# LCSL/nys-koop-lqr

Hardware: AMD Instinct MI355X
Metric: Nyström-Koopman fits/sec (K_nm build + A,B,C solve), N=1e5 m=2000 d=384 (higher is better)
Workload: dtype f64

## Files before the change

nys_koop_lqr_amd/csrc/nk_api.hip:

```cpp
#include "nk_common.h"
#include "nk_plant.h"

#include <cmath>
#include <cstdarg>
#include <cstdio>
#include <cstring>
#include <chrono>
#include <cstdlib>
#include <algorithm>
#include <condition_variable>
#include <functional>
#include <mutex>
#include <set>
#include <thread>

namespace nk {

static thread_local std::string g_err;

void set_error(const char* fmt, ...) {
  char buf[1024];
  va_list ap;
  va_start(ap, fmt);
  vsnprintf(buf, sizeof(buf), fmt, ap);
// ... 1357 lines not shown
      double *Res = nullptr, *ResT = nullptr, *partial = nullptr;
      const int64_t ldt_ = nr + (nr & 1);
      NK_TRY(arena_alloc_t(ctx, (size_t)nr * mq, &Res));
      NK_TRY(arena_alloc_t(ctx, (size_t)mq * ldt_, &ResT));
      NK_TRY(arena_alloc_t(ctx, (size_t)2 * refine_partial_blocks(), &partial));
      CholSys y = sys[q];
      y.R = ResT; y.ldr = ldt_; y.nrhs = nr;
      for (int step = 0; step < refine_steps; ++step) {
        NK_TRY(launch_resid_dd(ctx, Xq, mq, Pq, mq, Rq, mq, Res, mq, nr, mq));
        NK_TRY(launch_transpose(ctx, Res, mq, ResT, ldt_, nr, mq));
        NK_TRY(cholesky_solve_pair(ctx, &y, 1));
        NK_TRY(launch_transpose(ctx, ResT, ldt_, Res, mq, mq, nr));
        NK_TRY(launch_refine_apply(ctx, Res, mq, Xq, mq, nr, mq, step, refine_state + 4 * q, partial));
      }
      NK_HIP(hipMemcpyAsync(ctx->h_scalars + 16 + 4 * q, refine_state + 4 * q, 4 * sizeof(double), hipMemcpyDeviceToHost,
                            ctx->stream));
      arena_release(ctx, mk);
      refined[q] = -1;
      redo_products = true;
    }
  }
  {
    const int vr = sqrtm_verdict(ctx, &splan, &it, &resid);
    if (vr == NK_SQRT_RETRY && splan.flow_gave_up) {
      ChainOnly chain(ctx);
      SqrtPlan again;
      again.lambda_min_hint = splan.lambda_min_hint;
      NK_TRY(sqrtm_prepare(ctx, Kj, m, m, &again));
      NK_TRY(sqrtm_finish(ctx, &again, mdl->S, mdl->Sinv));
      NK_HIP(hipStreamSynchronize(ctx->stream));
      const int vr2 = sqrtm_verdict(ctx, &again, &it, &resid);
      if (vr2 == NK_SQRT_RETRY) {
        count_event(CNT_SQRT_RETRY);
        NK_TRY(sqrtm_spd_coupled(ctx, Kj, m, m, mdl->S, mdl->Sinv, &it, &resid));
      } else {
        NK_TRY(vr2);
      }
      NK_TRY(sqrt_products());
      redo_products = true;
    } else if (vr == NK_SQRT_RETRY) {
      count_event(CNT_SQRT_RETRY);
      NK_TRY(sqrtm_spd_coupled(ctx, Kj, m, m, mdl->S, mdl->Sinv, &it, &resid));
      NK_TRY(sqrt_products());
      redo_products = true;
    } else {
      NK_TRY(vr);
    }
// ... 1207 lines not shown
```

nys_koop_lqr_amd/csrc/nk_common.h:

```cpp
#pragma once
#include <hip/hip_runtime.h>
#include <stdint.h>
#include <stddef.h>
#include <string>
#include <vector>

#include "nyskoop.h"
#include "nk_lockstep.h"

namespace nk {

void set_error(const char* fmt, ...);

#define NK_HIP(call)                                                                         \
  do {                                                                                       \
    hipError_t e_ = (call);                                                                  \
    if (e_ != hipSuccess) {                                                                  \
      nk::set_error("%s failed: %s (%s:%d)", #call, hipGetErrorString(e_), __FILE__, __LINE__); \
      return e_ == hipErrorOutOfMemory ? NK_ERR_OOM : NK_ERR_HIP;                            \
    }                                                                                        \
  } while (0)

#define NK_TRY(call)            \
  do {                          \
// ... 166 lines not shown
  const double z = s * s;
  const double w = z * z;
  const double t1 = w * (Lg2 + w * (Lg4 + w * Lg6));
  const double t2 = z * (Lg1 + w * (Lg3 + w * (Lg5 + w * Lg7)));
  const double R = t2 + t1;
  if (((hx - 0x6147a) | (0x6b851 - hx)) > 0) {
    const double hfsq = 0.5 * f * f;
    return k == 0 ? f - (hfsq - s * (hfsq + R)) : dk * ln2_hi - ((hfsq - (s * (hfsq + R) + dk * ln2_lo)) - f);
  }
  return k == 0 ? f - s * (f - R) : dk * ln2_hi - ((s * (f - R) - dk * ln2_lo) - f);
}
__host__ __device__ __forceinline__ double tps_value(double r2) {
#pragma clang fp contract(off)
  return r2 > 0.0 ? r2 * log_pos(sqrt(r2)) : 0.0;
}

nk_group* group_new(int device, int size);
void group_attach(nk_group* g, int slot, nk_ctx* c);
void group_detach(nk_ctx* c);
int group_enter(nk_ctx* c);
int group_leave(nk_ctx* c);
void group_stats(nk_ctx* c, uint64_t out[4]);
enum { CNT_CHAIN_GIVEUP = 0, CNT_JACOBI_GIVEUP = 1, CNT_RANK_TRUNCATED = 2, CNT_SQRT_RETRY = 3, CNT_REFINED = 4,
       CNT_CHOL_FLOW_GIVEUP = 5, CNT_CHOL_FLOW = 6, CNT_N = 7 };
void count_event(int which);
uint64_t read_counter(int which);
hipError_t real_stream_sync(hipStream_t s);
hipError_t real_event_sync(hipEvent_t e);

int arena_reset(nk_ctx* ctx);
ArenaMark arena_mark(nk_ctx* ctx);
void arena_release(nk_ctx* ctx, ArenaMark mk);
int arena_alloc(nk_ctx* ctx, size_t bytes, void** out);
template <typename T>
inline int arena_alloc_t(nk_ctx* ctx, size_t count, T** out) {
  return arena_alloc(ctx, count * sizeof(T), reinterpret_cast<void**>(out));
}
bool is_device_ptr(const void* p);

int launch_kmat(nk_ctx* ctx, int ktype, const double* A, int64_t lda, int64_t nA, const double* B, int64_t ldb,
                int64_t nB, int d, const double* winv, double sigma0, double* out, int64_t ldo);

enum { TRI_FULL = 0, TRI_UPPER_MIRROR = 1, TRI_LOWER = 2 };
struct GemmOpts {
  int tri = TRI_FULL;
  int splitk = 0;
};
// ... 24 lines not shown
                               const TnSkip* skip = nullptr);
int launch_max_abs_rowsum(nk_ctx* ctx, const double* M, int64_t ldm, int n, double* d_out);
int launch_colsum_sqdiff(nk_ctx* ctx, const double* P, int64_t ldp, const double* Y, int64_t ldy, int64_t rows,
                         int cols, double* d_colsum);

int sqrtm_spd(nk_ctx* ctx, const double* P, int64_t ldp, int m, double* S, double* Sinv, int* iters, double* resid);
struct SqrtPlan {
  const double* P = nullptr;
  int64_t ldp = 0;
  int m = 0;
  double* W = nullptr;
  double* Linv = nullptr;
  double* X0 = nullptr;
  double* X0t = nullptr;
  double* d_sc = nullptr;
  ArenaMark mark{0, 0};
  bool deferred = false;
  int rc = 0, iters = 0, kmax = 0;
  double resid = 0.0;
  double lambda_min_hint = 0.0;
  bool early = false;
  int info_slot = 2;
  bool flow_gave_up = false;
  hipEvent_t pause_event = nullptr;
  int pause_step = -1;
};
constexpr int NK_SQRT_RETRY = 1;
int sqrtm_spd_coupled(nk_ctx* ctx, const double* P, int64_t ldp, int m, double* S, double* Sinv, int* iters, double* resid);
int sqrtm_prepare(nk_ctx* ctx, const double* P, int64_t ldp, int m, SqrtPlan* plan);
int sqrtm_finish(nk_ctx* ctx, SqrtPlan* plan, double* S, double* Sinv);
int sqrtm_verdict(nk_ctx* ctx, SqrtPlan* plan, int* iters, double* resid);
int cholesky_lower(nk_ctx* ctx, double* P, int64_t ldp, int m, double* Linv );
int cholesky_solve(nk_ctx* ctx, const double* L, int64_t ldl, int m, const double* Linv, double* R, int64_t ldr,
                   int nrhs);
struct CholSys {
  double* P = nullptr;
  int64_t ldp = 0;
  int m = 0;
  int extra = 0;
  bool backward = true;
  double* Linv = nullptr;
  double* pivlog = nullptr;
  double* R = nullptr;
  int64_t ldr = 0;
  int nrhs = 0;
};
int cholesky_lower_pair(nk_ctx* ctx, const CholSys* sys, int nsys);
int cholesky_lower_pair_async(nk_ctx* ctx, const CholSys* sys, int nsys);
int cholesky_check_pair(nk_ctx* ctx, const CholSys* sys, int nsys);
int cholesky_solve_pair(nk_ctx* ctx, const CholSys* sys, int nsys);
int cholesky_aug_pair_async(nk_ctx* ctx, const CholSys* sys, int nsys, hipEvent_t pause = nullptr, int pause_step = -1);
constexpr int CHOL_NB = 64;
constexpr int CHOL_WS = 2 * CHOL_NB * CHOL_NB + 8;
constexpr double CHOL_FIX_KAPPA = 8.0 * CHOL_NB;
// ... 63 lines not shown
  const double* A = nullptr;
  const double* B = nullptr;
  double* C = nullptr;
  int64_t lda = 0, ldb = 0, ldc = 0;
  int M = 0, N = 0;
  int tri = TRI_FULL;
  int ktrim = 0;
  double alpha = 1.0, beta = 0.0;
  double* Ct = nullptr;
  int64_t ldct = 0;
  const double* A_even = nullptr;
  const double* B_even = nullptr;
  double* Caff = nullptr;
  double aff_a = 0.0, aff_c = 0.0;
};
struct TnSkip {
  const double* state = nullptr;
  int step = 0;
  const double* select = nullptr;
  double* resid_partials = nullptr;
  int* resid_count = nullptr;
};
bool tn_fast_ok(const TnProblem& p);
struct TnProblemF {
  const float* A = nullptr;
  const float* B = nullptr;
  double* C = nullptr;
  int64_t lda = 0, ldb = 0, ldc = 0;
  int M = 0, N = 0;
  int tri = TRI_FULL;
  double beta = 0.0;
};
bool tnf_fast_ok(const TnProblemF& p);
int launch_gemm_tn_f32_multi(nk_ctx* ctx, const TnProblemF* probs, int nprob, int64_t K, int splitk ,
                             float* ms_kernel = nullptr, bool sync_timing = true);
int prep_rows_f32(nk_ctx* ctx, const double* X, int64_t ldx, int64_t rows, int d, const double* winv, const double* center,
                  float* Xt, int64_t ldt, float* sq);
int launch_cvt_f64_f32(nk_ctx* ctx, const double* src, int64_t lds_, float* dst, int64_t ldd, int64_t rows, int cols);
int launch_kmat_gram_f32(nk_ctx* ctx, int ktype, const float* At, int64_t ldat, const float* sqa, int64_t nA, const float* Bt,
                         int64_t ldbt, const float* sqb, int64_t nB, int d, double sigma0, float* out, int64_t ldo);
int launch_gemm_tn_multi(nk_ctx* ctx, const TnProblem* probs, int nprob, int64_t K, int splitk ,
                         float* ms_kernel = nullptr, bool sync_timing = true, const TnSkip* skip = nullptr);
int launch_transpose(nk_ctx* ctx, const double* src, int64_t lds, double* dst, int64_t ldd, int rows, int cols);
constexpr int refine_partial_blocks() { return 512; }
int launch_refine_apply(nk_ctx* ctx, const double* dX, int64_t ldd, double* X, int64_t ldx, int64_t rows, int64_t cols, int step,
                        double* state, double* partial);
// ... 56 lines not shown
```

nys_koop_lqr_amd/csrc/nk_gemm_tn.hip:

```cpp
#include "nk_common.h"
#include "nk_tn_kstep.inc"
#include "nk_tn_shared.h"

#include <cstdlib>
#include <cstring>

namespace nk {

typedef double d4 __attribute__((ext_vector_type(4)));

constexpr int TBK = 16;
constexpr int TSTRIDE = 144;
constexpr int TSTAGE = 2 * TBK * TSTRIDE;
constexpr int TN_LDS_BYTES = 2 * TSTAGE * 8;

struct TnDev {
  const double* A;
  const double* B;
  int64_t lda, ldb;
  int M, N;
  int tiles_n;
  int tri;
  int ktrim;
  int tile_begin;
// ... 399 lines not shown
    const int orow = bx + r, ocol = by + tx;
    if (orow < cols && ocol < rows) dst[(int64_t)orow * ldd + ocol] = tile[tx][r];
  }
}
__global__ void __launch_bounds__(256) transpose_kernel(const double* __restrict__ src, int64_t lds_, double* __restrict__ dst, int64_t ldd, int rows, int cols) { transpose_kernel_body(src, lds_, dst, ldd, rows, cols); }
NK_BATCHED_TWIN(transpose_kernel, (256), const double*, int64_t, double*, int64_t, int, int)

int launch_transpose(nk_ctx* ctx, const double* src, int64_t lds_, double* dst, int64_t ldd, int rows, int cols) {
  if (rows <= 0 || cols <= 0) return NK_OK;
  dim3 grid((cols + 31) / 32, (rows + 31) / 32);
  hipLaunchKernelGGL(transpose_kernel, grid, dim3(256), 0, ctx->stream, src, lds_, dst, ldd, rows, cols);
  NK_HIP(hipGetLastError());
  return NK_OK;
}

static inline bool aligned16(const void* p) { return (reinterpret_cast<uintptr_t>(p) & 15) == 0; }

bool tn_fast_ok(const TnProblem& p) {
  return p.M >= 2 && p.N >= 2 && aligned16(p.A) && aligned16(p.B) && p.lda % 2 == 0 && p.ldb % 2 == 0 &&
         p.lda >= ((p.M + 1) & ~1) && p.ldb >= ((p.N + 1) & ~1);
}

static bool g_tn_attr_set = false;
static int tn_use_asm() {
  const char* e = getenv("NYSKOOP_TN_ASM");
  return (e && e[0] == '0') ? 0 : 1;
}

int tn_ensure_zero_page(nk_ctx* ctx) {
  if (ctx->d_zeros) return NK_OK;
  NK_HIP(hipMalloc(reinterpret_cast<void**>(&ctx->d_zeros), 4096));
  NK_HIP(hipMemset(ctx->d_zeros, 0, 4096));
  return NK_OK;
}

int launch_gemm_tn_multi(nk_ctx* ctx, const TnProblem* probs, int nprob, int64_t K, int splitk, float* ms_kernel,
                         bool sync_timing, const TnSkip* skip) {
  NK_REQUIRE(nprob >= 1 && nprob <= TN_MAXP, "gemm_tn_multi: 1..4 problems");
  NK_REQUIRE(K >= 0 && K < (1LL << 31), "gemm_tn_multi: K out of range");
  NK_TRY(tn_ensure_zero_page(ctx));
  TnParams P;
  TnRedParams R;
  int ntiles = 0;
  for (int q = 0; q < nprob; ++q) {
    const TnProblem& s = probs[q];
    NK_REQUIRE(tn_fast_ok(s), "gemm_tn_multi: problem %d violates the alignment contract", q);
    NK_REQUIRE(s.tri == TRI_FULL || (s.tri == TRI_UPPER_MIRROR && s.M == s.N), "gemm_tn_multi: bad tri mode");
    const int tmn = (s.M + TBM - 1) / TBM, tnn = (s.N + TBM - 1) / TBM;
    TnDev& d = P.p[q];
    d.A = s.A; d.B = s.B; d.lda = s.lda; d.ldb = s.ldb; d.M = s.M; d.N = s.N;
    d.tiles_n = tnn; d.tri = s.tri; d.ktrim = s.ktrim; d.tile_begin = ntiles;
    d.C = s.C; d.ldc = s.ldc; d.alpha = s.alpha; d.beta = s.beta; d.Ct = s.Ct; d.ldct = s.ldct;
    d.A_even = s.A_even; d.B_even = s.B_even;
    d.Caff = s.Caff; d.aff_a = s.aff_a; d.aff_c = s.aff_c;
    TnRed& r = R.p[q];
    r.Caff = s.Caff; r.aff_a = s.aff_a; r.aff_c = s.aff_c;
    r.Ct = s.Ct; r.ldct = s.ldct;
    r.C = s.C; r.ldc = s.ldc; r.M = s.M; r.N = s.N; r.tiles_n = tnn; r.tri = s.tri; r.tile_begin = ntiles;
    r.alpha = s.alpha; r.beta = s.beta;
    ntiles += s.tri == TRI_FULL ? tmn * tnn : tmn * (tmn + 1) / 2;
  }
  for (int q = nprob; q < TN_MAXP; ++q) {
    P.p[q] = P.p[0];
    P.p[q].tile_begin = 1 << 30;
    R.p[q] = R.p[0];
    R.p[q].tile_begin = 1 << 30;
  }
  const int ktiles_total = (int)((K + TBK - 1) / TBK);
  const bool want_resid = skip && skip->resid_partials != nullptr;
  if (splitk <= 0) {
    const int slots = 2 * ctx->num_cu;
    const int max_split = ktiles_total / 8 > 1 ? ktiles_total / 8 : 1;
    double best = 1e300;
    splitk = 1;
    for (int c = 1; c <= 64 && c <= max_split; ++c) {
      const int64_t wgs = (int64_t)ntiles * c;
      const double steps = (double)((ktiles_total + c - 1) / c);
      const int64_t full = wgs / slots, rem = wgs % slots;
      double t = full * 2.44 * steps;
      if (rem > 0) t += (rem <= ctx->num_cu ? 2.35 : 2.44) * steps;
      t *= 4096.0;
      if (c > 1) t += (double)wgs * (TBM * TBM * 8.0 * 2.0) / 4.0e12 * 2.4e9;
      t += 2000.0 * c / 8.0;
      if (c % 8 == 0) t *= 0.97;
      if (t < best) { best = t; splitk = c; }
    }
  }
  if (want_resid && splitk < 2) splitk = 2;
  if (nprob >= 3 && getenv("NYSKOOP_TN_SPLITK")) splitk = atoi(getenv("NYSKOOP_TN_SPLITK"));
  P.kmask = getenv("NYSKOOP_TN_KMASK") ? (int)strtol(getenv("NYSKOOP_TN_KMASK"), nullptr, 0) : -1;
  P.use_asm = tn_use_asm();
  P.nprob = nprob; P.ntiles = ntiles; P.K = (int)K; P.splitk = splitk;
  P.klen = ((ktiles_total + splitk - 1) / splitk) * TBK;
  if (P.klen == 0) P.klen = TBK;
  P.zeros = ctx->d_zeros;
  const ArenaMark mark = arena_mark(ctx);
  double* slab = nullptr;
  if (splitk > 1) NK_TRY(arena_alloc_t(ctx, (size_t)ntiles * splitk * TBM * TBM, &slab));
  P.slab = slab;
  R.nprob = nprob; R.splitk = splitk; R.slab = slab;
  P.skip_state = R.skip_state = skip ? skip->state : nullptr;
  P.skip_step = R.skip_step = skip ? skip->step : 0;
  P.select_state = skip ? skip->select : nullptr;
  R.resid_partials = (skip && splitk > 1 && nprob == 1) ? skip->resid_partials : nullptr;
  if (skip && skip->resid_count) *skip->resid_count = R.resid_partials ? ntiles * RPARTS : 0;
  if (!g_tn_attr_set) {
    NK_HIP(hipFuncSetAttribute(reinterpret_cast<const void*>(gemm_tn_f64_kernel<0>),
                               hipFuncAttributeMaxDynamicSharedMemorySize, TN_LDS_BYTES));
    NK_HIP(hipFuncSetAttribute(reinterpret_cast<const void*>(gram_fused_f64_kernel),
                               hipFuncAttributeMaxDynamicSharedMemorySize, TN_LDS_BYTES));
// ... 187 lines not shown
```

nys_koop_lqr_amd/csrc/nk_linalg.hip:

```cpp
#include "nk_common.h"

#include <algorithm>
#include <cmath>
#include <cstring>
#include <vector>

namespace nk {

__device__ __forceinline__ void add_diag_kernel_body(double* A, int64_t lda, int n, double v) {
  int i = blockIdx.x * blockDim.x + threadIdx.x;
  if (i < n) A[(int64_t)i * lda + i] += v;
}
__global__ void __launch_bounds__(256) add_diag_kernel(double* A, int64_t lda, int n, double v) { add_diag_kernel_body(A, lda, n, v); }
NK_BATCHED_TWIN(add_diag_kernel, (256), double*, int64_t, int, double)
__device__ __forceinline__ void copy2d_kernel_body(const double* __restrict__ src, int64_t lds, double* __restrict__ dst, int64_t ldd, int64_t rows, int64_t cols) {
  const int64_t total = rows * cols;
  for (int64_t e = blockIdx.x * (int64_t)blockDim.x + threadIdx.x; e < total; e += (int64_t)gridDim.x * blockDim.x) {
    const int64_t r = e / cols, c = e - r * cols;
    dst[r * ldd + c] = src[r * lds + c];
  }
}
__global__ void __launch_bounds__(256) copy2d_kernel(const double* __restrict__ src, int64_t lds, double* __restrict__ dst, int64_t ldd, int64_t rows, int64_t cols) { copy2d_kernel_body(src, lds, dst, ldd, rows, cols); }
NK_BATCHED_TWIN(copy2d_kernel, (256), const double*, int64_t, double*, int64_t, int64_t, int64_t)
__device__ __forceinline__ void axpby2d_kernel_body(double a, const double* __restrict__ X, int64_t ldx, double b, double* __restrict__ Y, int64_t ldy, int64_t rows, int64_t cols) {
// ... 855 lines not shown
    double v = 0.0;
    if (i < m && j <= i) v = L[(int64_t)i * ldl + j] * s;
    if (i < m && j < m) Xt[(int64_t)i * m + j] = v;
    tile[r][tx] = v;
  }
  __syncthreads();
  for (int r = ty; r < 32; r += 8) {
    const int i = bx + r, j = by + tx;
    if (i < m && j < m) X[(int64_t)i * m + j] = tile[tx][r];
  }
}
__global__ void __launch_bounds__(256) tri_scale_both_kernel(const double* __restrict__ L, int64_t ldl, int m, const double* __restrict__ d_c, double* __restrict__ Xt, double* __restrict__ X) { tri_scale_both_kernel_body(L, ldl, m, d_c, Xt, X); }
NK_BATCHED_TWIN(tri_scale_both_kernel, (256), const double*, int64_t, int, const double*, double*, double*)

int sqrtm_prepare(nk_ctx* ctx, const double* P, int64_t ldp, int m, SqrtPlan* plan) {
  plan->P = P; plan->ldp = ldp; plan->m = m;
  plan->mark = arena_mark(ctx);
  const size_t mm = (size_t)m * m;
  const int nblk = (m + CHOL_NB - 1) / CHOL_NB;
  NK_TRY(arena_alloc_t(ctx, 2 * mm, &plan->W));
  NK_TRY(arena_alloc_t(ctx, (size_t)nblk * CHOL_WS, &plan->Linv));
  NK_TRY(arena_alloc_t(ctx, mm, &plan->X0));
  NK_TRY(arena_alloc_t(ctx, mm, &plan->X0t));
  NK_TRY(arena_alloc_t(ctx, (size_t)8, &plan->d_sc));
  NK_TRY(launch_max_abs_rowsum(ctx, P, ldp, m, plan->d_sc));
  {
    const ArenaMark mk = arena_mark(ctx);
    const int blocks = grid_for((int64_t)m * m, ctx->num_cu);
    double* partial = nullptr;
    NK_TRY(arena_alloc_t(ctx, (size_t)2 * blocks, &partial));
    hipLaunchKernelGGL(sumsq_trace_partial_kernel, dim3(blocks), dim3(256), 0, ctx->stream, P, ldp, m, partial, blocks);
    hipLaunchKernelGGL(sum_partials_kernel, dim3(1), dim3(256), 0, ctx->stream, partial, blocks, plan->d_sc + 1);
    hipLaunchKernelGGL(sum_partials_kernel, dim3(1), dim3(256), 0, ctx->stream, partial + blocks, blocks, plan->d_sc + 2);
    NK_HIP(hipGetLastError());
    arena_release(ctx, mk);
  }
  NK_HIP(hipMemcpyAsync(ctx->h_scalars + 12, plan->d_sc, 3 * sizeof(double), hipMemcpyDeviceToHost, ctx->stream));
  NK_HIP(hipEventRecord(ctx->ev[11], ctx->stream));
  double* E = plan->W + mm;
  NK_TRY(launch_copy2d(ctx, P, ldp, plan->W, m, m, m));
  NK_TRY(launch_fill(ctx, E, m, m, m, 0.0));
  NK_TRY(launch_add_diag(ctx, E, m, m, 1.0));
  CholSys y;
  y.P = plan->W; y.ldp = m; y.m = m; y.extra = m; y.backward = false; y.Linv = plan->Linv;
  NK_TRY(cholesky_aug_pair_async(ctx, &y, 1, plan->pause_event, plan->pause_step));
  {
    const ArenaMark mk = arena_mark(ctx);
// ... 131 lines not shown

  if (queued) {
    double s2s[128];
    bool checks[128];
    int kmax = 0;
    {
      double ta = plan->early ? 0.9 * plan->lambda_min_hint / c : 0.5 / (c * linv2), tb = 1.0;
      if (ta > a_lo) ta = a_lo;
      const double a_sched = std::pow(a_lo, 0.8) * std::pow(ta, 0.2);
      double a = a_sched, b = b_hi;
      int kconv = -1;
      for (int k = 0; k < 100; ++k) {
        if (kconv < 0 && ta >= 1.0 - 1e-9 && tb <= 1.0 + 1e-9) kconv = k;
        checks[k] = a >= 0.5;
        const double s2 = 3.0 / (a + std::sqrt(a * b) + b);
        s2s[k] = s2;
        advance(s2, a, b);
        advance(s2, ta, tb);
        if (kconv >= 0 && k >= kconv + 1) { kmax = k + 1; break; }
      }
      if (kmax == 0) kmax = 100;
    }
    double* state = plan->d_sc + 5;
    NK_HIP(hipMemsetAsync(state, 0, 3 * sizeof(double), ctx->stream));
    double* rpart = nullptr;
    {
      const size_t mt = (size_t)(m + 127) / 128;
      const size_t need = std::max((size_t)grid_for((int64_t)m * m, ctx->num_cu), mt * (mt + 1) / 2 * 8);
      NK_TRY(arena_alloc_t(ctx, need, &rpart));
    }
    for (int k = 0; k < kmax; ++k) {
      TnSkip skip;
      skip.state = state; skip.step = k;
      int npart = 0;
      if (k == 0) {
        NK_TRY(launch_transpose(ctx, plan->P, plan->ldp, M, m, m, m));
        NK_TRY(launch_axpby2d(ctx, 0.5 / c, plan->P, plan->ldp, 0.5 / c, M, m, m, m));
      } else {
        const double s2k = s2s[k], sck = std::sqrt(s2k);
        TnProblem pm;
        pm.A = X; pm.B = X; pm.C = M; pm.lda = pm.ldb = pm.ldc = m; pm.M = pm.N = m; pm.tri = TRI_UPPER_MIRROR;
        pm.Caff = T; pm.aff_a = -0.5 * s2k * sck; pm.aff_c = 1.5 * sck;
        TnSkip skip_m = skip;
        skip_m.resid_partials = rpart; skip_m.resid_count = &npart;
        NK_TRY(launch_gemm_tn_multi(ctx, &pm, 1, m, 0, nullptr, true, &skip_m));
      }
      if (checks[k]) {
        if (npart == 0) {
          npart = grid_for((int64_t)m * m, ctx->num_cu);
          hipLaunchKernelGGL(frob_mi_partial_kernel, dim3(npart), dim3(256), 0, ctx->stream, M, (int64_t)m, m, rpart,
                             skip.state, skip.step);
        }
        hipLaunchKernelGGL(ns_flag_kernel, dim3(1), dim3(256), 0, ctx->stream, rpart, npart, m, k, state);
        NK_HIP(hipGetLastError());
      }
      if (k == 0) {
        const double s2 = s2s[0], sc = std::sqrt(s2);
        NK_TRY(launch_scale_add_identity(ctx, -0.5 * s2 * sc, M, m, 1.5 * sc, T, m, m, &skip));
      }
      TnProblem pr;
      pr.A = Xt; pr.B = T; pr.C = Xn; pr.lda = pr.ldb = pr.ldc = m; pr.M = pr.N = m; pr.Ct = Xtn; pr.ldct = m;
      NK_TRY(launch_gemm_tn_multi(ctx, &pr, 1, m, 1, nullptr, true, &skip));
      X = Xn; Xt = Xtn;
      Xn = (Xn == Xa) ? Xb : Xa;
      Xtn = (Xtn == Xta) ? Xtb : Xta;
    }
    NK_TRY(sqrtm_polar_products(ctx, plan, Xa, T, c, S, Sinv, Xb, state));
    NK_HIP(hipMemcpyAsync(ctx->h_scalars + 8, state, 3 * sizeof(double), hipMemcpyDeviceToHost, ctx->stream));
    if (plan->early)
      NK_HIP(hipMemcpyAsync(ctx->h_info + ib, ctx->d_info + ib, sizeof(int), hipMemcpyDeviceToHost, ctx->stream));
    plan->deferred = true;
    plan->kmax = kmax;
    arena_release(ctx, plan->mark);
    return NK_OK;
  }

  const int maxit = 100;
  double r = 1e300;
  int it = 0;
  bool ok = false;
  for (; it < maxit; ++it) {
    if (it == 0) {
      NK_TRY(launch_transpose(ctx, plan->P, plan->ldp, M, m, m, m));
      NK_TRY(launch_axpby2d(ctx, 0.5 / c, plan->P, plan->ldp, 0.5 / c, M, m, m, m));
    } else {
      NK_TRY(launch_gemm(ctx, true, false, m, m, m, 1.0, X, m, X, m, 0.0, M, m, sym));
    }
    const bool check = a_lo >= 0.5 || it + 2 >= maxit;
    if (check) {
      NK_TRY(launch_frob_minus_identity(ctx, M, m, m, ctx->d_scalars));
      NK_HIP(hipMemcpyAsync(ctx->h_scalars, ctx->d_scalars, sizeof(double), hipMemcpyDeviceToHost, ctx->stream));
// ... 24 lines not shown
        break;
      }
    }
  }
  plan->iters = it;
  plan->resid = r;
  NK_TRY(x_align());
  if (!ok) {
    set_error("sqrtm: Newton-Schulz did not converge (residual %g after %d iterations)", r, it);
    arena_release(ctx, plan->mark);
    plan->rc = NK_ERR_NO_CONVERGENCE;
    return plan->rc;
  }
  NK_TRY(sqrtm_polar_products(ctx, plan, X, T, c, S, Sinv));
  arena_release(ctx, plan->mark);
  return NK_OK;
}

int sqrtm_verdict(nk_ctx* ctx, SqrtPlan* plan, int* iters, double* resid) {
  if (plan->deferred) {
    const double flag = ctx->h_scalars[8];
    plan->deferred = false;
    const int word = ctx->h_info[plan->info_slot];
    if (plan->early && (word != 0 || flag == 0.0 || !std::isfinite(ctx->h_scalars[10]))) {
      plan->flow_gave_up = word == CHOL_FLOW_GIVEUP;
      if (plan->flow_gave_up) count_event(CNT_CHOL_FLOW_GIVEUP);
      plan->iters = plan->kmax;
      plan->resid = ctx->h_scalars[10];
      plan->rc = NK_SQRT_RETRY;
    } else if (flag == 0.0 || !std::isfinite(ctx->h_scalars[10])) {
      plan->iters = plan->kmax;
      plan->resid = ctx->h_scalars[10];
      plan->rc = NK_ERR_NO_CONVERGENCE;
      set_error("sqrtm: Newton-Schulz did not converge (residual %g after %d iterations)", plan->resid, plan->kmax);
    } else {
      plan->iters = (int)flag;
      plan->resid = ctx->h_scalars[9];
      plan->rc = NK_OK;
    }
  }
  if (iters) *iters = plan->iters;
  if (resid) *resid = plan->resid;
  return plan->rc;
}

int sqrtm_spd(nk_ctx* ctx, const double* P, int64_t ldp, int m, double* S, double* Sinv, int* iters, double* resid) {
  SqrtPlan plan;
  NK_TRY(sqrtm_prepare(ctx, P, ldp, m, &plan));
  NK_TRY(sqrtm_finish(ctx, &plan, S, Sinv));
  NK_HIP(hipStreamSynchronize(ctx->stream));
  return sqrtm_verdict(ctx, &plan, iters, resid);
}

}
```

Before: 24.65.

## Run Newton-Schulz sqrtm iterations in one persistent dataflow kernel

Replaces the per-iteration sequence of SYRK, scale-add and TN GEMM launches in the matrix square root with a single persistent kernel. Work-groups pull tickets from an atomic counter and synchronise through per-tile flags, so later iterations can start on tiles whose inputs are ready instead of waiting at kernel boundaries. Split-K reduction and the convergence check also run on device, with an early-exit state. When the flow kernel gives up, a new flag sends control back to a full retry path, which adds complexity and a risk of spin-wait deadlocks or extra reruns.

```diff
diff --git a/nys_koop_lqr_amd/csrc/nk_api.hip b/nys_koop_lqr_amd/csrc/nk_api.hip
--- a/nys_koop_lqr_amd/csrc/nk_api.hip
+++ b/nys_koop_lqr_amd/csrc/nk_api.hip
@@ -1403,7 +1403,7 @@
   }
   {
     const int vr = sqrtm_verdict(ctx, &splan, &it, &resid);
-    if (vr == NK_SQRT_RETRY && splan.flow_gave_up) {
+    if (vr == NK_SQRT_RETRY && (splan.flow_gave_up || splan.sqrt_flow_gave_up)) {
       ChainOnly chain(ctx);
       SqrtPlan again;
       again.lambda_min_hint = splan.lambda_min_hint;
diff --git a/nys_koop_lqr_amd/csrc/nk_common.h b/nys_koop_lqr_amd/csrc/nk_common.h
--- a/nys_koop_lqr_amd/csrc/nk_common.h
+++ b/nys_koop_lqr_amd/csrc/nk_common.h
@@ -212,7 +212,7 @@
 int group_leave(nk_ctx* c);
 void group_stats(nk_ctx* c, uint64_t out[4]);
 enum { CNT_CHAIN_GIVEUP = 0, CNT_JACOBI_GIVEUP = 1, CNT_RANK_TRUNCATED = 2, CNT_SQRT_RETRY = 3, CNT_REFINED = 4,
-       CNT_CHOL_FLOW_GIVEUP = 5, CNT_CHOL_FLOW = 6, CNT_N = 7 };
+       CNT_CHOL_FLOW_GIVEUP = 5, CNT_CHOL_FLOW = 6, CNT_SQRT_FLOW = 7, CNT_SQRT_FLOW_GIVEUP = 8, CNT_N = 9 };
 void count_event(int which);
 uint64_t read_counter(int which);
 hipError_t real_stream_sync(hipStream_t s);
@@ -283,6 +283,7 @@
   bool early = false;
   int info_slot = 2;
   bool flow_gave_up = false;
+  bool sqrt_flow_gave_up = false;
   hipEvent_t pause_event = nullptr;
   int pause_step = -1;
 };
@@ -291,6 +292,21 @@
 int sqrtm_prepare(nk_ctx* ctx, const double* P, int64_t ldp, int m, SqrtPlan* plan);
 int sqrtm_finish(nk_ctx* ctx, SqrtPlan* plan, double* S, double* Sinv);
 int sqrtm_verdict(nk_ctx* ctx, SqrtPlan* plan, int* iters, double* resid);
+constexpr int SQRT_FLOW_MAX_STEPS = 100;
+struct SqrtFlowPlan {
+  int m = 0, kmax = 0;
+  const double* X0 = nullptr;
+  const double* X0t = nullptr;
+  double *Xa = nullptr, *Xta = nullptr, *Xb = nullptr, *Xtb = nullptr;
+  double* T = nullptr;
+  double* rpart = nullptr;
+  double* state = nullptr;
+  const double* aff_a = nullptr;
+  const double* aff_c = nullptr;
+  const bool* check = nullptr;
+};
+bool sqrt_flow_enabled();
+int sqrt_flow_iterate(nk_ctx* ctx, const SqrtFlowPlan& p);
 int cholesky_lower(nk_ctx* ctx, double* P, int64_t ldp, int m, double* Linv );
 int cholesky_solve(nk_ctx* ctx, const double* L, int64_t ldl, int m, const double* Linv, double* R, int64_t ldr,
                    int nrhs);
@@ -400,6 +416,8 @@
   int* resid_count = nullptr;
 };
 bool tn_fast_ok(const TnProblem& p);
+int tn_pick_splitk(const nk_ctx* ctx, int ntiles, int ktiles_total);
+int tn_use_asm();
 struct TnProblemF {
   const float* A = nullptr;
   const float* B = nullptr;
diff --git a/nys_koop_lqr_amd/csrc/nk_gemm_tn.hip b/nys_koop_lqr_amd/csrc/nk_gemm_tn.hip
--- a/nys_koop_lqr_amd/csrc/nk_gemm_tn.hip
+++ b/nys_koop_lqr_amd/csrc/nk_gemm_tn.hip
@@ -445,7 +445,7 @@
 }
 
 static bool g_tn_attr_set = false;
-static int tn_use_asm() {
+int tn_use_asm() {
   const char* e = getenv("NYSKOOP_TN_ASM");
   return (e && e[0] == '0') ? 0 : 1;
 }
@@ -455,6 +455,26 @@
   NK_HIP(hipMalloc(reinterpret_cast<void**>(&ctx->d_zeros), 4096));
   NK_HIP(hipMemset(ctx->d_zeros, 0, 4096));
   return NK_OK;
+}
+
+int tn_pick_splitk(const nk_ctx* ctx, int ntiles, int ktiles_total) {
+  const int slots = 2 * ctx->num_cu;
+  const int max_split = ktiles_total / 8 > 1 ? ktiles_total / 8 : 1;
+  double best = 1e300;
+  int splitk = 1;
+  for (int c = 1; c <= 64 && c <= max_split; ++c) {
+    const int64_t wgs = (int64_t)ntiles * c;
+    const double steps = (double)((ktiles_total + c - 1) / c);
+    const int64_t full = wgs / slots, rem = wgs % slots;
+    double t = full * 2.44 * steps;
+    if (rem > 0) t += (rem <= ctx->num_cu ? 2.35 : 2.44) * steps;
+    t *= 4096.0;
+    if (c > 1) t += (double)wgs * (TBM * TBM * 8.0 * 2.0) / 4.0e12 * 2.4e9;
+    t += 2000.0 * c / 8.0;
+    if (c % 8 == 0) t *= 0.97;
+    if (t < best) { best = t; splitk = c; }
+  }
+  return splitk;
 }
 
 int launch_gemm_tn_multi(nk_ctx* ctx, const TnProblem* probs, int nprob, int64_t K, int splitk, float* ms_kernel,
@@ -491,24 +511,7 @@
   }
   const int ktiles_total = (int)((K + TBK - 1) / TBK);
   const bool want_resid = skip && skip->resid_partials != nullptr;
-  if (splitk <= 0) {
-    const int slots = 2 * ctx->num_cu;
-    const int max_split = ktiles_total / 8 > 1 ? ktiles_total / 8 : 1;
-    double best = 1e300;
-    splitk = 1;
-    for (int c = 1; c <= 64 && c <= max_split; ++c) {
-      const int64_t wgs = (int64_t)ntiles * c;
-      const double steps = (double)((ktiles_total + c - 1) / c);
-      const int64_t full = wgs / slots, rem = wgs % slots;
-      double t = full * 2.44 * steps;
-      if (rem > 0) t += (rem <= ctx->num_cu ? 2.35 : 2.44) * steps;
-      t *= 4096.0;
-      if (c > 1) t += (double)wgs * (TBM * TBM * 8.0 * 2.0) / 4.0e12 * 2.4e9;
-      t += 2000.0 * c / 8.0;
-      if (c % 8 == 0) t *= 0.97;
-      if (t < best) { best = t; splitk = c; }
-    }
-  }
+  if (splitk <= 0) splitk = tn_pick_splitk(ctx, ntiles, ktiles_total);
   if (want_resid && splitk < 2) splitk = 2;
   if (nprob >= 3 && getenv("NYSKOOP_TN_SPLITK")) splitk = atoi(getenv("NYSKOOP_TN_SPLITK"));
   P.kmask = getenv("NYSKOOP_TN_KMASK") ? (int)strtol(getenv("NYSKOOP_TN_KMASK"), nullptr, 0) : -1;
diff --git a/nys_koop_lqr_amd/csrc/nk_linalg.hip b/nys_koop_lqr_amd/csrc/nk_linalg.hip
--- a/nys_koop_lqr_amd/csrc/nk_linalg.hip
+++ b/nys_koop_lqr_amd/csrc/nk_linalg.hip
@@ -901,7 +901,7 @@
   NK_TRY(arena_alloc_t(ctx, (size_t)nblk * CHOL_WS, &plan->Linv));
   NK_TRY(arena_alloc_t(ctx, mm, &plan->X0));
   NK_TRY(arena_alloc_t(ctx, mm, &plan->X0t));
-  NK_TRY(arena_alloc_t(ctx, (size_t)8, &plan->d_sc));
+  NK_TRY(arena_alloc_t(ctx, (size_t)16, &plan->d_sc));
   NK_TRY(launch_max_abs_rowsum(ctx, P, ldp, m, plan->d_sc));
   {
     const ArenaMark mk = arena_mark(ctx);
@@ -1079,7 +1079,9 @@
       if (kmax == 0) kmax = 100;
     }
     double* state = plan->d_sc + 5;
-    NK_HIP(hipMemsetAsync(state, 0, 3 * sizeof(double), ctx->stream));
+    NK_HIP(hipMemsetAsync(state, 0, 4 * sizeof(double), ctx->stream));
+    const bool flow = !ctx->chol_flow_off && !ctx_recording(ctx) && kmax <= SQRT_FLOW_MAX_STEPS && 2 * ((m + 127) / 128) <= 64 &&
+                      sqrt_flow_enabled();
     double* rpart = nullptr;
     {
       const size_t mt = (size_t)(m + 127) / 128;
@@ -1115,6 +1117,19 @@
         const double s2 = s2s[0], sc = std::sqrt(s2);
         NK_TRY(launch_scale_add_identity(ctx, -0.5 * s2 * sc, M, m, 1.5 * sc, T, m, m, &skip));
       }
+      if (flow) {
+        double aff_a[SQRT_FLOW_MAX_STEPS], aff_c[SQRT_FLOW_MAX_STEPS];
+        for (int j = 0; j < kmax; ++j) {
+          const double sj = std::sqrt(s2s[j]);
+          aff_a[j] = -0.5 * s2s[j] * sj;
+          aff_c[j] = 1.5 * sj;
+        }
+        SqrtFlowPlan fp;
+        fp.m = m; fp.kmax = kmax; fp.X0 = plan->X0; fp.X0t = plan->X0t; fp.Xa = Xa; fp.Xta = Xta; fp.Xb = Xb; fp.Xtb = Xtb;
+        fp.T = T; fp.rpart = rpart; fp.state = state; fp.aff_a = aff_a; fp.aff_c = aff_c; fp.check = checks;
+        NK_TRY(sqrt_flow_iterate(ctx, fp));
+        break;
+      }
       TnProblem pr;
       pr.A = Xt; pr.B = T; pr.C = Xn; pr.lda = pr.ldb = pr.ldc = m; pr.M = pr.N = m; pr.Ct = Xtn; pr.ldct = m;
       NK_TRY(launch_gemm_tn_multi(ctx, &pr, 1, m, 1, nullptr, true, &skip));
@@ -1123,7 +1138,7 @@
       Xtn = (Xtn == Xta) ? Xtb : Xta;
     }
     NK_TRY(sqrtm_polar_products(ctx, plan, Xa, T, c, S, Sinv, Xb, state));
-    NK_HIP(hipMemcpyAsync(ctx->h_scalars + 8, state, 3 * sizeof(double), hipMemcpyDeviceToHost, ctx->stream));
+    NK_HIP(hipMemcpyAsync(ctx->h_scalars + 8, state, 4 * sizeof(double), hipMemcpyDeviceToHost, ctx->stream));
     if (plan->early)
       NK_HIP(hipMemcpyAsync(ctx->h_info + ib, ctx->d_info + ib, sizeof(int), hipMemcpyDeviceToHost, ctx->stream));
     plan->deferred = true;
@@ -1194,7 +1209,13 @@
     const double flag = ctx->h_scalars[8];
     plan->deferred = false;
     const int word = ctx->h_info[plan->info_slot];
-    if (plan->early && (word != 0 || flag == 0.0 || !std::isfinite(ctx->h_scalars[10]))) {
+    plan->sqrt_flow_gave_up = ctx->h_scalars[11] != 0.0;
+    if (plan->sqrt_flow_gave_up) {
+      count_event(CNT_SQRT_FLOW_GIVEUP);
+      plan->iters = plan->kmax;
+      plan->resid = ctx->h_scalars[10];
+      plan->rc = NK_SQRT_RETRY;
+    } else if (plan->early && (word != 0 || flag == 0.0 || !std::isfinite(ctx->h_scalars[10]))) {
       plan->flow_gave_up = word == CHOL_FLOW_GIVEUP;
       if (plan->flow_gave_up) count_event(CNT_CHOL_FLOW_GIVEUP);
       plan->iters = plan->kmax;
@@ -1221,7 +1242,16 @@
   NK_TRY(sqrtm_prepare(ctx, P, ldp, m, &plan));
   NK_TRY(sqrtm_finish(ctx, &plan, S, Sinv));
   NK_HIP(hipStreamSynchronize(ctx->stream));
-  return sqrtm_verdict(ctx, &plan, iters, resid);
-}
-
-}
+  const int rc = sqrtm_verdict(ctx, &plan, iters, resid);
+  if (rc == NK_SQRT_RETRY && plan.sqrt_flow_gave_up) {
+    ChainOnly chain(ctx);
+    SqrtPlan again;
+    NK_TRY(sqrtm_prepare(ctx, P, ldp, m, &again));
+    NK_TRY(sqrtm_finish(ctx, &again, S, Sinv));
+    NK_HIP(hipStreamSynchronize(ctx->stream));
+    return sqrtm_verdict(ctx, &again, iters, resid);
+  }
+  return rc;
+}
+
+}
diff --git a/nys_koop_lqr_amd/csrc/nk_sqrt_flow.hip b/nys_koop_lqr_amd/csrc/nk_sqrt_flow.hip
--- /dev/null
+++ b/nys_koop_lqr_amd/csrc/nk_sqrt_flow.hip
@@ -0,0 +1,510 @@
+#include <cstdio>
+#include <cstdlib>
+#include <cstring>
+
+#include "nk_common.h"
+#include "nk_tn_kstep.inc"
+#include "nk_tn_shared.h"
+
+namespace nk {
+
+namespace {
+
+typedef double d4 __attribute__((ext_vector_type(4)));
+typedef double d2 __attribute__((ext_vector_type(2)));
+
+constexpr int TBK = 16;
+constexpr int TSTRIDE = 144;
+constexpr int TSTAGE = 2 * TBK * TSTRIDE;
+constexpr int TN_LDS_DOUBLES = 2 * TSTAGE;
+constexpr int SF_LDS_BYTES = TN_LDS_DOUBLES * 8 + 64;
+constexpr int SF_HDR = 16;
+constexpr int SF_POLL_LIMIT = 1 << 22;
+
+struct SqrtFlowArgs {
+  const double* X0;
+  const double* X0t;
+  double *Xa, *Xta;
+  double *Xb, *Xtb;
+  double* T;
+  double* slab;
+  double* rpart;
+  double* state;
+  const double* zeros;
+  int* hdr;
+  int* mflag;
+  int* xflag;
+  int* arrive;
+  int* reduced;
+  int* decided;
+  int m, nt, ntri, splitk, klen, kmax, total, use_asm, test_giveup;
+  double aff_a[SQRT_FLOW_MAX_STEPS], aff_c[SQRT_FLOW_MAX_STEPS];
+  signed char gate[SQRT_FLOW_MAX_STEPS];
+  unsigned char check[SQRT_FLOW_MAX_STEPS];
+};
+
+__device__ __forceinline__ int ld_flag(const int* f) { return __hip_atomic_load(f, __ATOMIC_RELAXED, __HIP_MEMORY_SCOPE_AGENT); }
+__device__ __forceinline__ double ld_state(const double* p) {
+  return __longlong_as_double((long long)__hip_atomic_load(reinterpret_cast<const unsigned long long*>(p), __ATOMIC_RELAXED,
+                                                           __HIP_MEMORY_SCOPE_AGENT));
+}
+
+__device__ __forceinline__ uint64_t uniform_u64(uint64_t v) {
+  return ((uint64_t)(uint32_t)__builtin_amdgcn_readfirstlane((uint32_t)(v >> 32)) << 32) |
+         (uint64_t)(uint32_t)__builtin_amdgcn_readfirstlane((uint32_t)v);
+}
+__device__ __forceinline__ void dma_row(const double* row_base, uint32_t lane_off_bytes, uint32_t lds_addr) {
+  const uint64_t rbu = uniform_u64((uint64_t)(uintptr_t)row_base);
+  asm volatile("s_mov_b32 m0, %2\n\ts_nop 0\n\tglobal_load_lds_dwordx4 %0, %1"
+               :
+               : "v"(lane_off_bytes), "s"(rbu), "s"((uint32_t)__builtin_amdgcn_readfirstlane(lds_addr))
+               : "m0");
+}
+__device__ __forceinline__ void dma_wait_all() { asm volatile("s_waitcnt vmcnt(0)" ::: "memory"); }
+
+__device__ __forceinline__ void tile_kloop(double* smem, const double* opA, int64_t lda, const double* opB, int64_t ldb, int M,
+                                           int N, int tm, int tn, int kbeg, int kend, const double* zeros, int use_asm,
+                                           d4 (&acc)[4][4]) {
+  const int lane = threadIdx.x & 63;
+  const int wave = __builtin_amdgcn_readfirstlane(threadIdx.x >> 6);
+  const int ktiles = kend > kbeg ? (kend - kbeg + TBK - 1) / TBK : 0;
+  const uint32_t offa = (uint32_t)min(tm * TBM + lane * 2, (M - 1) & ~1) * 8u;
+  const uint32_t offb = (uint32_t)min(tn * TBM + lane * 2, (N - 1) & ~1) * 8u;
+  const uint32_t offz = (uint32_t)lane * 16u;
+  const uint32_t lds0 = (uint32_t)(uintptr_t)smem;
+  auto issue = [&](int kt, int stage) {
+    const uint32_t sa = lds0 + (uint32_t)(stage * TSTAGE) * 8u;
+    const uint32_t sb = sa + (uint32_t)(TBK * TSTRIDE) * 8u;
+    const int k0 = kbeg + kt * TBK;
+    if (k0 + TBK <= kend) {
+#pragma unroll
+      for (int q = 0; q < 4; ++q) {
+        const int r = wave + 4 * q;
+        dma_row(opA + (int64_t)(k0 + r) * lda, offa, sa + (uint32_t)(r * TSTRIDE) * 8u);
+        dma_row(opB + (int64_t)(k0 + r) * ldb, offb, sb + (uint32_t)(r * TSTRIDE) * 8u);
+      }
+    } else {
+#pragma unroll
+      for (int q = 0; q < 4; ++q) {
+        const int r = wave + 4 * q;
+        const int k = k0 + r;
+        if (k < kend) {
+          dma_row(opA + (int64_t)k * lda, offa, sa + (uint32_t)(r * TSTRIDE) * 8u);
+          dma_row(opB + (int64_t)k * ldb, offb, sb + (uint32_t)(r * TSTRIDE) * 8u);
+        } else {
+          dma_row(zeros, offz, sa + (uint32_t)(r * TSTRIDE) * 8u);
+          dma_row(zeros, offz, sb + (uint32_t)(r * TSTRIDE) * 8u);
+        }
+      }
+    }
+  };
+#pragma unroll
+  for (int i = 0; i < 4; ++i)
+#pragma unroll
+    for (int j = 0; j < 4; ++j) acc[i][j] = d4{0.0, 0.0, 0.0, 0.0};
+  const int wm = wave >> 1, wn = wave & 1;
+  const int r16 = lane & 15, g4 = lane >> 4;
+  auto frag = [&](int stage, int ks, double (&a)[4], double (&b)[4]) {
+    const double* a_base = smem + stage * TSTAGE + wm * 64 + r16 + (ks * 4 + g4) * TSTRIDE;
+    const double* b_base = a_base + TBK * TSTRIDE + (wn - wm) * 64;
+#pragma unroll
+    for (int i = 0; i < 4; ++i) a[i] = a_base[i * 16];
+#pragma unroll
+    for (int j = 0; j < 4; ++j) b[j] = b_base[j * 16];
+  };
+  auto mma = [&](const double (&a)[4], const double (&b)[4]) {
+#pragma unroll
+    for (int i = 0; i < 4; ++i)
+#pragma unroll
+      for (int j = 0; j < 4; ++j) acc[i][j] = __builtin_amdgcn_mfma_f64_16x16x4f64(a[i], b[j], acc[i][j], 0, 0, 0);
+  };
+  double a0[4], b0[4], a1[4], b1[4];
+  if (ktiles > 0) {
+    issue(0, 0);
+    dma_wait_all();
+    __syncthreads();
+    frag(0, 0, a0, b0);
+  }
+  const uint32_t ard0 = lds0 + (uint32_t)(wm * 64 + r16 + g4 * TSTRIDE) * 8u;
+  const uint32_t brd0 = lds0 + (uint32_t)(TBK * TSTRIDE + wn * 64 + r16 + g4 * TSTRIDE) * 8u;
+  constexpr uint32_t STAGE_B = (uint32_t)TSTAGE * 8u;
+  const uint32_t stra = (uint32_t)__builtin_amdgcn_readfirstlane((uint32_t)(lda * 32));
+  const uint32_t strb = (uint32_t)__builtin_amdgcn_readfirstlane((uint32_t)(ldb * 32));
+  const int nfull = (kend - kbeg) / TBK;
+  int kt_start = 0;
+  if (use_asm && nfull >= 1) {
+    const uint32_t dst0 = (uint32_t)__builtin_amdgcn_readfirstlane(lds0 + (uint32_t)(wave * TSTRIDE) * 8u);
+    const uint32_t dst1 = dst0 + STAGE_B;
+    const uint32_t ard1 = ard0 + STAGE_B, brd1 = brd0 + STAGE_B;
+    const int steady = nfull - 1;
+    uint32_t cnt = (uint32_t)__builtin_amdgcn_readfirstlane((uint32_t)(steady / 2));
+    const uint32_t flags = (uint32_t)__builtin_amdgcn_readfirstlane((uint32_t)((steady & 1) | (nfull == ktiles ? 2 : 0)));
+    kt_start = 2 * (int)cnt + (int)(flags & 1) + (int)(flags >> 1);
+    const uint64_t rowa = uniform_u64((uint64_t)(uintptr_t)(opA + (int64_t)(kbeg + TBK + wave) * lda));
+    const uint64_t rowb = uniform_u64((uint64_t)(uintptr_t)(opB + (int64_t)(kbeg + TBK + wave) * ldb));
+    if (kt_start > 0)
+      asm volatile(NK_TN_KSTEPS_ASM
+                   : [c00] "+v"(acc[0][0]), [c01] "+v"(acc[0][1]), [c02] "+v"(acc[0][2]), [c03] "+v"(acc[0][3]),
+                     [c10] "+v"(acc[1][0]), [c11] "+v"(acc[1][1]), [c12] "+v"(acc[1][2]), [c13] "+v"(acc[1][3]),
+                     [c20] "+v"(acc[2][0]), [c21] "+v"(acc[2][1]), [c22] "+v"(acc[2][2]), [c23] "+v"(acc[2][3]),
+                     [c30] "+v"(acc[3][0]), [c31] "+v"(acc[3][1]), [c32] "+v"(acc[3][2]), [c33] "+v"(acc[3][3]),
+                     [a00] "+v"(a0[0]), [a01] "+v"(a0[1]), [a02] "+v"(a0[2]), [a03] "+v"(a0[3]), [b00] "+v"(b0[0]),
+                     [b01] "+v"(b0[1]), [b02] "+v"(b0[2]), [b03] "+v"(b0[3]), [a10] "=&v"(a1[0]), [a11] "=&v"(a1[1]),
+                     [a12] "=&v"(a1[2]), [a13] "=&v"(a1[3]), [b10] "=&v"(b1[0]), [b11] "=&v"(b1[1]), [b12] "=&v"(b1[2]),
+                     [b13] "=&v"(b1[3]), [cnt] "+s"(cnt)
+                   : [ard0] "v"(ard0), [brd0] "v"(brd0), [ard1] "v"(ard1), [brd1] "v"(brd1), [voa] "v"(offa), [vob] "v"(offb),
+                     [rowa] "s"(rowa), [rowb] "s"(rowb), [stra] "s"(stra), [strb] "s"(strb), [dst0] "s"(dst0),
+                     [dst1] "s"(dst1), [flags] "s"(flags)
+                   : "memory", "m0", "scc", "s92", "s93", "s94", "s95");
+  }
+  for (int kt = kt_start; kt < ktiles; ++kt) {
+    const int st = kt & 1;
+    const bool more = kt + 1 < ktiles;
+    frag(st, 1, a1, b1);
+    if (more) issue(kt + 1, st ^ 1);
+    mma(a0, b0);
+    __builtin_amdgcn_sched_barrier(0);
+    frag(st, 2, a0, b0);
+    __builtin_amdgcn_sched_barrier(0);
+    mma(a1, b1);
+    __builtin_amdgcn_sched_barrier(0);
+    frag(st, 3, a1, b1);
+    __builtin_amdgcn_sched_barrier(0);
+    mma(a0, b0);
+    __builtin_amdgcn_sched_barrier(0);
+    dma_wait_all();
+    __syncthreads();
+    if (more) frag(st ^ 1, 0, a0, b0);
+    __builtin_amdgcn_sched_barrier(0);
+    mma(a1, b1);
+    __builtin_amdgcn_sched_barrier(0);
+  }
+}
+
+__device__ __forceinline__ int tri_index(int tm, int tn, int nt) {
+  if ((nt & 7) == 0) {
+    const int S = nt >> 3, I = tm >> 3, J = tn >> 3, r = tm & 7, c = tn & 7;
+    int base = 0;
+    for (int i = 0; i < I; ++i) base += 36 + 64 * (S - 1 - i);
+    if (J > I) base += 36 + 64 * (J - I - 1);
+    return base + (I == J ? r * 8 - r * (r - 1) / 2 + (c - r) : r * 8 + c);
+  }
+  return tm * nt - tm * (tm - 1) / 2 + (tn - tm);
+}
+
+__device__ __forceinline__ void give_up(const SqrtFlowArgs& a) {
+  __hip_atomic_store(a.hdr + 1, 1, __ATOMIC_RELAXED, __HIP_MEMORY_SCOPE_AGENT);
+  __hip_atomic_store(reinterpret_cast<unsigned long long*>(a.state + 3), (unsigned long long)__double_as_longlong(1.0),
+                     __ATOMIC_RELAXED, __HIP_MEMORY_SCOPE_AGENT);
+}
+
+__device__ int wait_flags(const SqrtFlowArgs& a, const int* f, int* ctl, int step = -1) {
+  if (threadIdx.x < 64) {
+    int res = 0;
+    for (int polls = 0;; ++polls) {
+      const bool ok = f == nullptr || ld_flag(f) != 0;
+      if (__all(ok)) { res = 1; break; }
+      if (step >= 0) {
+        const double c = ld_state(a.state);
+        if (__any(c != 0.0 && c <= (double)step)) { res = 2; break; }
+      }
+      if (ld_flag(a.hdr + 1) != 0) break;
+      if (polls >= SF_POLL_LIMIT) {
+        if (threadIdx.x == 0) give_up(a);
+        break;
+      }
+      __builtin_amdgcn_s_sleep(2);
+    }
+    if (threadIdx.x == 0) {
+      if (res) __builtin_amdgcn_fence(__ATOMIC_ACQUIRE, "agent");
+      asm volatile("s_waitcnt vmcnt(0)" ::: "memory");
+      ctl[0] = res;
+    }
+  }
+  __syncthreads();
+  const int r = ctl[0];
+  __syncthreads();
+  return r;
+}
+
+__device__ __forceinline__ void release_all() {
+  asm volatile("s_waitcnt vmcnt(0)" ::: "memory");
+  __syncthreads();
+  if (threadIdx.x == 0) {
+    __builtin_amdgcn_fence(__ATOMIC_RELEASE, "agent");
+    asm volatile("s_waitcnt vmcnt(0)" ::: "memory");
+  }
+}
+
+__device__ __forceinline__ void reduce_tile(const SqrtFlowArgs& a, int gt, int tm, int tn, double aff_a, double aff_c,
+                                            double* sh, double* wsum) {
+  const bool mirror = tm != tn;
+  const int m = a.m;
+  for (int part = 0; part < RPARTS; ++part) {
+    const double* base = a.slab + (int64_t)gt * a.splitk * (TBM * TBM) + part * (16 * TBM) + threadIdx.x * 2;
+    d2 s[4];
+#pragma unroll
+    for (int i = 0; i < 4; ++i) s[i] = d2{0.0, 0.0};
+    for (int k = 0; k < a.splitk; ++k) {
+      const double* bk = base + (int64_t)k * (TBM * TBM);
+#pragma unroll
+      for (int i = 0; i < 4; ++i) s[i] += *reinterpret_cast<const d2*>(bk + 512 * i);
+    }
+    const int row0 = tm * TBM + part * 16, col0 = tn * TBM;
+    double rsum = 0.0;
+#pragma unroll
+    for (int i = 0; i < 4; ++i) {
+      const int idx = threadIdx.x * 2 + 512 * i;
+      const int r = idx >> 7, c = idx & 127;
+      const int row = row0 + r;
+#pragma unroll
+      for (int h = 0; h < 2; ++h) {
+        const int col = col0 + c + h;
+        double v = 0.0;
+        if (row < m && col < m) {
+          v = s[i][h];
+          a.T[(int64_t)row * m + col] = aff_a * v + (row == col ? aff_c : 0.0);
+          const double e = v - (row == col ? 1.0 : 0.0);
+          rsum = fma(e, e, rsum);
+        }
+        if (mirror) sh[r * 130 + c + h] = v;
+      }
+    }
+#pragma unroll
+    for (int off = 32; off > 0; off >>= 1) rsum += __shfl_down(rsum, off, 64);
+    if ((threadIdx.x & 63) == 0) wsum[threadIdx.x >> 6] = rsum;
+    __syncthreads();
+    if (threadIdx.x == 0) {
+      const double w = (wsum[0] + wsum[1]) + (wsum[2] + wsum[3]);
+      a.rpart[gt * RPARTS + part] = mirror ? 2.0 * w : w;
+    }
+    if (mirror) {
+      const int c = threadIdx.x >> 1, rb = (threadIdx.x & 1) * 8;
+      const int col = col0 + c;
+      if (col < m) {
+#pragma unroll
+        for (int q = 0; q < 8; ++q) {
+          const int row = row0 + rb + q;
+          if (row >= m) break;
+          a.T[(int64_t)col * m + row] = aff_a * sh[(rb + q) * 130 + c];
+        }
+      }
+    }
+    __syncthreads();
+  }
+}
+
+__device__ __forceinline__ void decide(const SqrtFlowArgs& a, int step, double* wsum) {
+  const int count = a.ntri * RPARTS;
+  double s = 0.0;
+  for (int i = threadIdx.x; i < count; i += 256) s += a.rpart[i];
+#pragma unroll
+  for (int off = 32; off > 0; off >>= 1) s += __shfl_down(s, off, 64);
+  if ((threadIdx.x & 63) == 0) wsum[threadIdx.x >> 6] = s;
+  __syncthreads();
+  if (threadIdx.x == 0) {
+    const double r = sqrt((wsum[0] + wsum[1] + wsum[2] + wsum[3]) / a.m);
+    a.state[2] = r;
+    if (ld_state(a.state) == 0.0 && r < 1e-7) {
+      a.state[0] = (double)(step + 1);
+      a.state[1] = r;
+    }
+    asm volatile("s_waitcnt vmcnt(0)" ::: "memory");
+    __builtin_amdgcn_fence(__ATOMIC_RELEASE, "agent");
+    asm volatile("s_waitcnt vmcnt(0)" ::: "memory");
+    __hip_atomic_store(a.decided + step, 1, __ATOMIC_RELAXED, __HIP_MEMORY_SCOPE_AGENT);
+  }
+  __syncthreads();
+}
+
+__global__ void __launch_bounds__(256, 2) sqrt_flow_kernel(SqrtFlowArgs a) {
+  extern __shared__ __attribute__((aligned(16))) double smem[];
+  int* ctl = reinterpret_cast<int*>(smem + TN_LDS_DOUBLES);
+  double* wsum = smem + TN_LDS_DOUBLES + 2;
+  const int lane = threadIdx.x & 63;
+  const int wave = __builtin_amdgcn_readfirstlane(threadIdx.x >> 6);
+  const int wm = wave >> 1, wn = wave & 1;
+  const int r16 = lane & 15, g4 = lane >> 4;
+  const int nt = a.nt, m = a.m;
+  const int nfull = nt * nt, nsy = a.ntri * a.splitk, per = nsy + nfull;
+  for (;;) {
+    if (threadIdx.x == 0) ctl[1] = atomicAdd(a.hdr, 1);
+    __syncthreads();
+    const int t = ctl[1];
+    __syncthreads();
+    if (t >= a.total) return;
+    if (t == a.test_giveup) {
+      if (threadIdx.x == 0) give_up(a);
+      return;
+    }
+    int step = 0, v = t;
+    if (t >= nfull) {
+      step = 1 + (t - nfull) / per;
+      v = (t - nfull) % per;
+    }
+    const int gate = a.gate[step];
+    if (gate >= 0 && wait_flags(a, lane == 0 ? a.decided + gate : nullptr, ctl, step) != 1) return;
+    if (threadIdx.x == 0) {
+      const double f = ld_state(a.state);
+      ctl[2] = ld_flag(a.hdr + 1) != 0 || (f != 0.0 && f <= (double)step);
+    }
+    __syncthreads();
+    const int leave = ctl[2];
+    __syncthreads();
+    if (leave) return;
+    const double* X = step == 0 ? a.X0 : ((step & 1) ? a.Xa : a.Xb);
+    const double* Xt = step == 0 ? a.X0t : ((step & 1) ? a.Xta : a.Xtb);
+    const bool syrk = step > 0 && v < nsy;
+    int gt = 0, split = 0, tm, tn;
+    const int* f = nullptr;
+    if (syrk) {
+      gt = v / a.splitk;
+      split = v - gt * a.splitk;
+      tn_tile_coords(gt, TRI_UPPER_MIRROR, nt, m, tm, tn);
+      if (lane < 2 * nt) f = a.xflag + (size_t)(step - 1) * nfull + (lane < nt ? tm : tn) * nt + (lane < nt ? lane : lane - nt);
+    } else {
+      const int pidx = step > 0 ? v - nsy : v;
+      tn = pidx / nt;
+      tm = pidx - tn * nt;
+      if (step > 0) {
+        if (lane < nt) f = a.mflag + (size_t)step * a.ntri + tri_index(min(lane, tn), max(lane, tn), nt);
+        else if (lane < 2 * nt) f = a.xflag + (size_t)(step - 1) * nfull + (lane - nt) * nt + tm;
+      }
+    }
+    if (step > 0 && !wait_flags(a, f, ctl)) return;
+    d4 acc[4][4];
+    {
+      const int kbeg = syrk ? split * a.klen : 0, kend = syrk ? min(m, kbeg + a.klen) : m;
+      tile_kloop(smem, syrk ? X : Xt, m, syrk ? X : a.T, m, m, m, tm, tn, kbeg, kend, a.zeros, a.use_asm, acc);
+    }
+    if (syrk) {
+      double* out = a.slab + ((int64_t)gt * a.splitk + split) * (TBM * TBM);
+#pragma unroll
+      for (int i = 0; i < 4; ++i)
+#pragma unroll
+        for (int j = 0; j < 4; ++j)
+#pragma unroll
+          for (int reg = 0; reg < 4; ++reg) {
+            const int row = wm * 64 + i * 16 + g4 + 4 * reg;
+            const int col = wn * 64 + j * 16 + r16;
+            out[row * TBM + col] = acc[i][j][reg];
+          }
+      release_all();
+      if (threadIdx.x == 0) {
+        const int old = __hip_atomic_fetch_add(a.arrive + (size_t)step * a.ntri + gt, 1, __ATOMIC_RELAXED, __HIP_MEMORY_SCOPE_AGENT);
+        const int last = old == a.splitk - 1;
+        if (last) __builtin_amdgcn_fence(__ATOMIC_ACQUIRE, "agent");
+        asm volatile("s_waitcnt vmcnt(0)" ::: "memory");
+        ctl[2] = last;
+      }
+      __syncthreads();
+      const int last = ctl[2];
+      __syncthreads();
+      if (!last) continue;
+      reduce_tile(a, gt, tm, tn, a.aff_a[step], a.aff_c[step], smem, wsum);
+      release_all();
+      if (threadIdx.x == 0) {
+        __hip_atomic_store(a.mflag + (size_t)step * a.ntri + gt, 1, __ATOMIC_RELAXED, __HIP_MEMORY_SCOPE_AGENT);
+        int fin = 0;
+        if (a.check[step]) {
+          const int old = __hip_atomic_fetch_add(a.reduced + step, 1, __ATOMIC_RELAXED, __HIP_MEMORY_SCOPE_AGENT);
+          fin = old == a.ntri - 1;
+          if (fin) __builtin_amdgcn_fence(__ATOMIC_ACQUIRE, "agent");
+          asm volatile("s_waitcnt vmcnt(0)" ::: "memory");
+        }
+        ctl[2] = fin;
+      }
+      __syncthreads();
+      const int fin = ctl[2];
+      __syncthreads();
+      if (fin) decide(a, step, wsum);
+    } else {
+      double* Xn = (step & 1) ? a.Xb : a.Xa;
+      double* Xtn = (step & 1) ? a.Xtb : a.Xta;
+#pragma unroll
+      for (int i = 0; i < 4; ++i)
+#pragma unroll
+        for (int j = 0; j < 4; ++j)
+#pragma unroll
+          for (int reg = 0; reg < 4; ++reg) {
+            const int row = tm * TBM + wm * 64 + i * 16 + g4 + 4 * reg;
+            const int col = tn * TBM + wn * 64 + j * 16 + r16;
+            if (row < m && col < m) {
+              const double x = acc[i][j][reg];
+              Xn[(int64_t)row * m + col] = x;
+              Xtn[(int64_t)col * m + row] = x;
+            }
+          }
+      release_all();
+      if (threadIdx.x == 0)
+        __hip_atomic_store(a.xflag + (size_t)step * nfull + tn * nt + tm, 1, __ATOMIC_RELAXED, __HIP_MEMORY_SCOPE_AGENT);
+    }
+  }
+}
+
+}
+
+bool sqrt_flow_enabled() {
+  const char* e = getenv("NYSKOOP_SQRT_FLOW");
+  return !(e && e[0] == '0');
+}
+
+static int sqrt_flow_test_giveup(int total) {
+  const char* e = getenv("NYSKOOP_SQRT_FLOW_TEST_GIVEUP");
+  if (!e || !e[0]) return -1;
+  long ticket = -1;
+  if (sscanf(e, "%ld", &ticket) < 1) return -1;
+  return (ticket >= 0 && ticket < total) ? (int)ticket : -1;
+}
+
+int sqrt_flow_iterate(nk_ctx* ctx, const SqrtFlowPlan& p) {
+  NK_REQUIRE(p.kmax >= 1 && p.kmax <= SQRT_FLOW_MAX_STEPS && p.m >= 128, "sqrt_flow_iterate: bad shape");
+  NK_TRY(tn_ensure_zero_page(ctx));
+  SqrtFlowArgs a;
+  memset(&a, 0, sizeof(a));
+  const int m = p.m, nt = (m + TBM - 1) / TBM, ntri = nt * (nt + 1) / 2, nfull = nt * nt;
+  NK_REQUIRE(2 * nt <= 64, "sqrt_flow_iterate: at most 32 tile rows");
+  a.X0 = p.X0; a.X0t = p.X0t; a.Xa = p.Xa; a.Xta = p.Xta; a.Xb = p.Xb; a.Xtb = p.Xtb; a.T = p.T; a.rpart = p.rpart;
+  a.state = p.state; a.zeros = ctx->d_zeros;
+  a.m = m; a.nt = nt; a.ntri = ntri; a.kmax = p.kmax;
+  const int ktiles_total = (m + TBK - 1) / TBK;
+  a.splitk = std::max(2, tn_pick_splitk(ctx, ntri, ktiles_total));
+  a.klen = ((ktiles_total + a.splitk - 1) / a.splitk) * TBK;
+  a.use_asm = tn_use_asm();
+  a.total = nfull + (p.kmax - 1) * (ntri * a.splitk + nfull);
+  a.test_giveup = sqrt_flow_test_giveup(a.total);
+  int gate = -1;
+  for (int k = 0; k < p.kmax; ++k) {
+    a.aff_a[k] = p.aff_a[k]; a.aff_c[k] = p.aff_c[k];
+    a.check[k] = p.check[k] ? 1 : 0;
+    a.gate[k] = (signed char)gate;
+    if (k >= 1 && p.check[k]) gate = k;
+  }
+  const ArenaMark mark = arena_mark(ctx);
+  NK_TRY(arena_alloc_t(ctx, (size_t)ntri * a.splitk * TBM * TBM, &a.slab));
+  size_t words = SF_HDR + (size_t)p.kmax * (2 * ntri + nfull + 2);
+  words = (words + 3) & ~(size_t)3;
+  NK_TRY(arena_alloc_t(ctx, words, &a.hdr));
+  a.mflag = a.hdr + SF_HDR;
+  a.xflag = a.mflag + (size_t)p.kmax * ntri;
+  a.arrive = a.xflag + (size_t)p.kmax * nfull;
+  a.reduced = a.arrive + (size_t)p.kmax * ntri;
+  a.decided = a.reduced + p.kmax;
+  NK_HIP(hipMemsetAsync(a.hdr, 0, words * sizeof(int), ctx->stream));
+  static bool attr_set = false;
+  if (!attr_set) {
+    NK_HIP(hipFuncSetAttribute(reinterpret_cast<const void*>(sqrt_flow_kernel), hipFuncAttributeMaxDynamicSharedMemorySize,
+                               SF_LDS_BYTES));
+    attr_set = true;
+  }
+  const char* se = getenv("NYSKOOP_SQRT_FLOW_SLOTS");
+  const int slots = (se && se[0] == '2') ? 2 : 1;
+  const int grid = std::max(1, std::min(a.total, slots * ctx->num_cu));
+  hipLaunchKernelGGL(sqrt_flow_kernel, dim3((unsigned)grid), dim3(256), SF_LDS_BYTES, ctx->stream, a);
+  NK_HIP(hipGetLastError());
+  count_event(CNT_SQRT_FLOW);
+  arena_release(ctx, mark);
+  return NK_OK;
+}
+
+}
```

After: 23.31. 0.946x the previous value.
